# flo-audio/flo

Measured on AMD Instinct MI355X. Metric: Msamples/s encoded (44.1k stereo, q=high), higher is better.
Workload: dtype f32

## Files before the change

### flo_amd/csrc/batch.cpp

```cpp
#include <algorithm>
#include <chrono>
#include <cstdio>
#include <cstdlib>
#include <cstring>

#include "batch_internal.hpp"
#include "container_kernels.hpp"
#include "devpool.hpp"
#include "lossy_kernels.hpp"

static size_t lossy_max_frame_bytes(int ch) { return 12 + 50 * (size_t)ch + (size_t)ch * (4 + 2064); }

static LossyPlan lossy_plan(const flo_batch *b, int which, int force_path) {
    const char *tc = getenv("FLO_TAIL_CRC"), *clips = getenv("FLO_CHAIN2X_CLIPS");
    return plan_lossy({.which = which, .force_path = force_path, .ch = b->ch, .n_clips = b->n_clips, .total_frames = b->total_frames,
                       .exact = lossy_exact(b->exact != 0, b->ts->dev), .in_coeffs = b->d_in_coeffs != nullptr, .debug = b->d_dbg_coeffs || b->d_dbg_q || b->d_dbg_sfw,
                       .dirty = b->ts->dev.dirty, .tail_crc = !(tc && tc[0] == '0'), .chain2q_clips = clips ? atoi(clips) : 0});
}
static int alloc_frame_scratch(flo_batch *b, const LossyPlan &p) {
    flo_ctx *c = b->ctx;
    if (p.form != LossyForm::Frames || b->d_at || !b->total_frames) return FLO_OK;
    const size_t n = (size_t)b->total_frames * b->ch * 32 * sizeof(float);
    HIPCHK(c, pool_alloc(&b->d_at, n));
    HIPCHK(c, pool_alloc(&b->d_sprev, n));
// ... 312 lines not shown
    F.channels = b->ch;
    F.bit_depth = 16;
    F.level = 5;
    F.n_clips = (int)b->n_clips;
    F.crc_out = b->d_crc;
    F.part_reg = b->d_part;
    if (P.crc_ready) {
        F.crc_ready = b->d_crc_ready;
        F.epoch = b->epoch;
    }
    F.max_frames = max_frames;
    if ((rc = timed_launch(c, "finish_files", [&] { return launch_finish_files(F, fin, c->stream); })) != FLO_OK) return rc;
    if (P.crc_ready) {
        if (!b->pin_sizes) {
            std::string perr;
            if (!(b->pin_sizes = (uint64_t *)stager_pinned_get(c->stager, b->n_clips * 8, perr))) return fail(c, FLO_ERR_NOMEM, perr);
        }
        HIPCHK(c, hipMemcpyAsync(b->pin_sizes, b->d_clip_bytes, b->n_clips * 8, hipMemcpyDeviceToHost, c->stream));
        b->sizes_queued = true;
    }
    return FLO_OK;
}

extern "C" int flo_batch_encode(flo_batch *b, int which) {
    if (!b) return FLO_ERR_ARG;
    flo_ctx *c = b->ctx;
    if (which < 0 || which > 5) return fail(c, FLO_ERR_ARG, "unknown kernel form");
    HIPCHK(c, hipSetDevice(c->device));
    b->encoded = false;
    b->synced = false;
    if (b->mode == FLO_MODE_LOSSY) b->plan = lossy_plan(b, which, c->force_path);
    int erc = batch_encode_launch(b);
    b->encoded = erc == FLO_OK;
    b->encode_failed = erc != FLO_OK;
    return erc;
}

#ifdef FLO_STAMPS
static int stamps_report(flo_batch *b) {
    flo_ctx *c = b->ctx;
    if (!b->d_stamps || b->plan.form != LossyForm::Chain2q) return FLO_OK;
    std::vector<unsigned long long> st(b->n_clips * 2 * 16);
    HIPCHK(c, hipMemcpy(st.data(), b->d_stamps, st.size() * 8, hipMemcpyDeviceToHost));
    double t[14] = {0}, p[14] = {0};
    for (size_t k = 0; k < b->n_clips; k++)
        for (int i = 0; i < 14; i++) { t[i] += (double)st[(2 * k) * 16 + i]; p[i] += (double)st[(2 * k + 1) * 16 + i]; }
    static const char *tn[] = {"fold", "prefetch", "fft", "postrot", "bandstats", "mask", "quant", "wait-consumed", "handover"};
    static const char *pn[] = {"wait-ready", "read/quant", "pack0", "pack1", "flush", "wait-ts"};
    fprintf(stderr, "[stamps2x] ticks (10 ns) per stereo frame | T:");
    double tt = 0, pt = 0;
    for (int i = 0; i < 9; i++) { fprintf(stderr, " %s=%.1f", tn[i], t[i] / b->total_frames); tt += t[i]; }
    fprintf(stderr, " total=%.1f | P:", tt / b->total_frames);
    for (int i = 0; i < 6; i++) { fprintf(stderr, " %s=%.1f", pn[i], p[i] / b->total_frames); pt += p[i]; }
    fprintf(stderr, " total=%.1f item-form declined %.4f of channel-frames", pt / b->total_frames, p[6] / (2.0 * b->total_frames));
    fprintf(stderr, " | T waits>1000: %.2f%% of frames, %.0f cyc/frame avg; >5000: %.2f%%, %.0f | P busy>12000: %.2f%%, %.0f; >20000: %.2f%%, %.0f\n",
            100 * t[10] / b->total_frames, t[9] / b->total_frames, 100 * t[12] / b->total_frames, t[11] / b->total_frames,
            100 * p[10] / b->total_frames, p[9] / b->total_frames, 100 * p[12] / b->total_frames, p[11] / b->total_frames);
    std::vector<double> pb(b->n_clips), tb(b->n_clips);
    for (size_t k = 0; k < b->n_clips; k++) {
        const double fr = (double)b->hops[k] > 0 ? (double)b->hops[k] : 1.0;
        double tq = 0, pq = 0;
        for (int i = 0; i < 9; i++) if (i != 7) tq += (double)st[(2 * k) * 16 + i];
        for (int i = 1; i < 5; i++) pq += (double)st[(2 * k + 1) * 16 + i];
        tb[k] = tq / fr; pb[k] = pq / fr;
    }
    if (const char *dump = getenv("FLO_STAMPS_DUMP")) {
        if (FILE *fh = fopen(dump, "wb")) {
            fwrite(st.data(), 8, st.size(), fh);
            fclose(fh);
        }
    }
    std::vector<double> ps = pb, ts = tb;
    std::sort(ps.begin(), ps.end()); std::sort(ts.begin(), ts.end());
    fprintf(stderr, "[stamps2x] per-clip busy ticks per frame, deciles | P:");
    for (int d = 0; d <= 10; d++) fprintf(stderr, " %.0f", ps[std::min(b->n_clips - 1, (size_t)(d * (b->n_clips - 1) / 10))]);
    fprintf(stderr, " | T:");
    for (int d = 0; d <= 10; d++) fprintf(stderr, " %.0f", ts[std::min(b->n_clips - 1, (size_t)(d * (b->n_clips - 1) / 10))]);
    size_t pbound = 0;
    for (size_t k = 0; k < b->n_clips; k++) pbound += pb[k] > tb[k];
    fprintf(stderr, " | clips whose packer is busier than their transform: %.1f%%\n", 100.0 * pbound / b->n_clips);
    return FLO_OK;
}
#else
static int stamps_report(flo_batch *) { return FLO_OK; }
#endif

static int batch_sync_impl(flo_batch *b, hipEvent_t done) {
    flo_ctx *c = b->ctx;
    HIPCHK(c, hipSetDevice(c->device));
    if (done) HIPCHK(c, hipEventSynchronize(done));
    else HIPCHK(c, hipStreamSynchronize(c->stream));
    if (!b->encoded && b->encode_failed) return fail(c, FLO_ERR_STATE, "the last flo_batch_encode on this batch failed");
    if (b->encoded && !b->synced) {
        if (b->mode == FLO_MODE_LOSSY) {
            b->h_clip_bytes.assign(b->n_clips, 0);
            b->h_frame_size.clear();
            if (b->sizes_queued) {
                memcpy(b->h_clip_bytes.data(), b->pin_sizes, b->n_clips * 8);
            } else if (b->n_clips && b->total_frames) {
                if (done && c->down_stream) {
                    HIPCHK(c, hipMemcpyAsync(b->h_clip_bytes.data(), b->d_clip_bytes, b->n_clips * 8, hipMemcpyDeviceToHost, c->down_stream));
                    HIPCHK(c, hipStreamSynchronize(c->down_stream));
                } else {
                    HIPCHK(c, hipMemcpy(b->h_clip_bytes.data(), b->d_clip_bytes, b->n_clips * 8, hipMemcpyDeviceToHost));
                }
            }
            for (size_t i = 0; i < b->n_clips; i++)
// ... 365 lines not shown
```

### flo_amd/csrc/lossy_device.hpp

```cpp
#pragma once
#include <hip/hip_runtime.h>
#include <stdint.h>

#include "pack_rows.h"

namespace flo {


struct LossyDevTables {
    const float4 *pack;
    const float4 *pack_g;
    const float4 *pack_ext;
    const float *ath_db;
    const uint8_t *band;
    const float *band_count;
    const float *s10d;
    const uint32_t *lane_bnd;
    const uint32_t *lane_slot0;
    const uint32_t *band_slot0;
    int max_band_slots;
    uint32_t dirty;
    float smr_thr;
    int q_transparent;
};
// ... 1060 lines not shown
                                           const QuantRows &R, uint32_t (&xs)[2][8]) {
    typedef float v4f __attribute__((ext_vector_type(4)));
    typedef __attribute__((address_space(3))) v4f lds_f4;
    const uint32_t ts0 = (uint32_t)__builtin_amdgcn_readfirstlane((int)(uint32_t)(uintptr_t)ts);
    const uint32_t sgn_mask = 0x7FFFFFFFu;
    uint32_t phalf = 0x3EFFFFFFu;
    asm volatile("" : "+v"(phalf));
#pragma unroll
    for (int g = 0; g < 4; g++) {
        const float4 al4 = T.pack[(kRowAth + g) * 64 + lane];
        const float4 bo4 = R.bo4[g];
        const float al[4] = {al4.x, al4.y, al4.z, al4.w};
        const uint32_t bo[4] = {__float_as_uint(bo4.x), __float_as_uint(bo4.y), __float_as_uint(bo4.z), __float_as_uint(bo4.w)};
        v4f tb[4];
#pragma unroll
        for (int k = 0; k < 4; k++) tb[k] = *reinterpret_cast<const lds_f4 *>((uintptr_t)(ts0 + 2u * bo[k]));
        int v[2][4];
        float t[2][4];
#pragma unroll
        for (int k = 0; k < 4; k++) {
            const v2f x = c[4 * g + k];
            const v2f xsc = x * (v2f){tb[k].z, tb[k].w};
            uint32_t h0, h1;
            asm("v_bfi_b32 %0, %1, %2, %3" : "=v"(h0) : "s"(sgn_mask), "v"(phalf), "v"(x.x));
            asm("v_bfi_b32 %0, %1, %2, %3" : "=v"(h1) : "s"(sgn_mask), "v"(phalf), "v"(x.y));
            const v2f rs = xsc + (v2f){__uint_as_float(h0), __uint_as_float(h1)};
            v[0][k] = cvt_rz(rs.x);
            v[1][k] = cvt_rz(rs.y);
            t[0][k] = max_raw(tb[k].x, al[k]);
            t[1][k] = max_raw(tb[k].y, al[k]);
        }
#pragma unroll
        for (int ch = 0; ch < 2; ch++)
#pragma unroll
            for (int k2 = 0; k2 < 2; k2++) {
                const float xe = ch ? c[4 * g + 2 * k2].y : c[4 * g + 2 * k2].x;
                const float xo = ch ? c[4 * g + 2 * k2 + 1].y : c[4 * g + 2 * k2 + 1].x;
                uint32_t r;
                asm("v_cmp_gt_f32_e64 vcc, |%1|, %2\n\t"
                    "v_cndmask_b32_e32 %0, 0, %3, vcc\n\t"
                    "v_cmp_gt_f32_e64 vcc, |%4|, %5\n\t"
                    "v_cndmask_b32_sdwa %0, 0, %6, vcc dst_sel:WORD_1 dst_unused:UNUSED_PRESERVE src0_sel:DWORD src1_sel:DWORD"
                    : "=&v"(r)
                    : "v"(xe), "v"(t[ch][2 * k2]), "v"(v[ch][2 * k2]), "v"(xo), "v"(t[ch][2 * k2 + 1]), "v"(v[ch][2 * k2 + 1])
                    : "vcc");
                xs[ch][2 * g + k2] = r;
            }
    }
}

typedef float v4f __attribute__((ext_vector_type(4)));
template <int TSOFF>
__device__ __forceinline__ void quantise_nat(const v4f (&cf)[8], const uint32_t (&ts_a)[16], const float (&athn)[16],
                                             const uint32_t alive, const uint32_t (&blk)[8], uint32_t (&xd)[2][8]) {
    typedef __attribute__((address_space(3))) v4f lds_f4;
    const uint32_t sgn_mask = 0x7FFFFFFFu;
    uint32_t phalf = 0x3EFFFFFFu;
    asm volatile("" : "+v"(phalf));
    auto block = [&](const int k, const v4f t0, const v4f t1, uint32_t &out0, uint32_t &out1) __attribute__((always_inline)) {
        const v2f x0 = {cf[k].x, cf[k].y}, x1 = {cf[k].z, cf[k].w};
        const v2f s0 = x0 * (v2f){t0.z, t0.w}, s1 = x1 * (v2f){t1.z, t1.w};
        uint32_t h00, h01, h10, h11;
        asm("v_bfi_b32 %0, %1, %2, %3" : "=v"(h00) : "s"(sgn_mask), "v"(phalf), "v"(x0.x));
        asm("v_bfi_b32 %0, %1, %2, %3" : "=v"(h01) : "s"(sgn_mask), "v"(phalf), "v"(x0.y));
        asm("v_bfi_b32 %0, %1, %2, %3" : "=v"(h10) : "s"(sgn_mask), "v"(phalf), "v"(x1.x));
        asm("v_bfi_b32 %0, %1, %2, %3" : "=v"(h11) : "s"(sgn_mask), "v"(phalf), "v"(x1.y));
        const v2f r0 = s0 + (v2f){__uint_as_float(h00), __uint_as_float(h01)};
        const v2f r1 = s1 + (v2f){__uint_as_float(h10), __uint_as_float(h11)};
        const int v0[2] = {cvt_rz(r0.x), cvt_rz(r0.y)}, v1[2] = {cvt_rz(r1.x), cvt_rz(r1.y)};
        const float a0 = athn[2 * k], a1 = athn[2 * k + 1];
        const float th0[2] = {max_raw(t0.x, a0), max_raw(t0.y, a0)}, th1[2] = {max_raw(t1.x, a1), max_raw(t1.y, a1)};
        uint32_t r[2];
#pragma unroll
        for (int ch = 0; ch < 2; ch++) {
            const float xe = ch ? x0.y : x0.x, xo = ch ? x1.y : x1.x;
            asm("v_cmp_gt_f32_e64 vcc, |%1|, %2\n\t"
                "v_cndmask_b32_e32 %0, 0, %3, vcc\n\t"
                "v_cmp_gt_f32_e64 vcc, |%4|, %5\n\t"
                "v_cndmask_b32_sdwa %0, 0, %6, vcc dst_sel:WORD_1 dst_unused:UNUSED_PRESERVE src0_sel:DWORD src1_sel:DWORD"
                : "=&v"(r[ch])
                : "v"(xe), "v"(th0[ch]), "v"(v0[ch]), "v"(xo), "v"(th1[ch]), "v"(v1[ch])
                : "vcc");
        }
        out0 = r[0];
        out1 = r[1];
    };
#pragma unroll
    for (int g = 0; g < 4; g++) {
        uint32_t o00 = 0u, o01 = 0u, o10 = 0u, o11 = 0u;
        if (alive & (blk[2 * g] | blk[2 * g + 1])) {
            v4f tb[4];
#pragma unroll
            for (int j = 0; j < 4; j++) tb[j] = *reinterpret_cast<const lds_f4 *>((uintptr_t)(ts_a[4 * g + j] + (uint32_t)TSOFF));
            if (alive & blk[2 * g]) block(2 * g, tb[0], tb[1], o00, o01);
            if (alive & blk[2 * g + 1]) block(2 * g + 1, tb[2], tb[3], o10, o11);
        }
        xd[0][2 * g] = o00, xd[1][2 * g] = o01;
        xd[0][2 * g + 1] = o10, xd[1][2 * g + 1] = o11;
    }
}

__device__ __forceinline__ uint32_t nonzero_mask16(const int (&q)[16]) {
    uint32_t m = 0;
#pragma unroll
    for (int e = 0; e < 16; e++) m |= (q[e] != 0 ? 1u : 0u) << e;
    return m;
}
__device__ __forceinline__ uint32_t nonzero_mask16_packed(const uint32_t (&x)[8], const uint32_t (&hi)[8]) {
    uint32_t m = 0;
#pragma unroll
    for (int k = 0; k < 8; k++) {
        m |= ((x[k] & 0xFFFFu) != 0u ? 1u : 0u) << (2 * k);
        m |= (hi[k] != 0u ? 1u : 0u) << (2 * k + 1);
    }
    return m;
}
__device__ __forceinline__ uint32_t wave_incl_sum(uint32_t x) {
    int v = (int)x;
    v += dpp_i<0x111>(0, v);
    v += dpp_i<0x112>(0, v);
    v += dpp_i<0x114>(0, v);
    v += dpp_i<0x118>(0, v);
    v += dpp_i<0x142, 0xA>(0, v);
    v += dpp_i<0x143, 0xC>(0, v);
    return (uint32_t)v;
}

struct SparsePlan {
    uint32_t M;
    int nn;
    int nz_end;
    uint32_t cross_cnt;
    uint32_t off0;
    uint32_t total;
};

__device__ __forceinline__ void sparse_plan_m(const int lane, const uint32_t m, SparsePlan &P) {
    const uint32_t prev_m = (uint32_t)dpp_i<0x138>(0, (int)m);
    const uint32_t prev_nz = (prev_m >> 15) & 1u;
    uint32_t zs = ~m & ((m << 1) | prev_nz) & 0xFFFFu;
    if (lane == 0 && !(m & 1u)) zs |= 1u;
    const int base = 16 * lane;
    const uint32_t inv = ~m & 0xFFFFu;
    const int first_nz = m ? base + __builtin_ctz(m) : 1024;
    const int first_z = inv ? base + __builtin_ctz(inv) : 1024;
    const int last_z = inv ? base + 31 - __builtin_clz(inv) : -1;
    const unsigned long long has_nz = __ballot(m != 0u), has_z = __ballot(inv != 0u);
    const unsigned long long nz_above = (has_nz >> 1) >> lane, z_above = (has_z >> 1) >> lane;
// ... 86 lines not shown
    while (any) {
        any = 0;
#pragma unroll
        for (int c = 0; c < CH; c++) {
            const bool active = CH == 1 || hm[c] != 0u;
            const int s = __builtin_ctz(hm[c] | 0x10000u);
            hm[c] &= hm[c] - 1;
            any |= hm[c];
            const uint32_t below = (1u << s) - 1u;
            const uint32_t off = P[c].off0 + 2u * (uint32_t)__builtin_popcount(P[c].M & (below | (below << 16)));
            const uint32_t above = m[c] >> s;
            const bool leaves = above == 0u;
            const int zin = (int)__builtin_ctz(above | 0x10000u);
            const uint32_t zc = leaves ? (uint32_t)(nn_rel[c] - s) : (uint32_t)zin;
            const int e = s + zin;
            const int run = __builtin_ctz(~(m[c] >> (e & 15)));
            const int len = (e + run >= 16) ? nzend_rel[c] - e : run;
            uint32_t cnt = (uint32_t)(len < 255 ? len : 255);
            cnt = leaves ? P[c].cross_cnt : cnt;
            const bool wide = zc >= 128u;
            const uint32_t o = active ? off : trash_off[c];
            dst[c][o] = (uint8_t)(wide ? ((zc & 0x7Fu) | 0x80u) : zc);
            dst[c][o + 1] = (uint8_t)(wide ? (zc >> 7) : cnt);
            dst[c][(wide && active) ? off + 2 : trash_off[c]] = (uint8_t)cnt;
        }
    }
#pragma unroll
    for (int i = 0; i < 16; i++) {
#pragma unroll
        for (int c = 0; c < CH; c++) {
            const uint32_t K = ((1u << i) - 1u) | (((2u << i) - 1u) << 16);
            const uint32_t off = P[c].off0 + 2u * (uint32_t)__builtin_popcount(P[c].M & K);
            const uint32_t o = ((m[c] >> i) & 1u) ? off : trash_off[c];
            const uint32_t v = (uint32_t)q[c][i];
            dst[c][o] = (uint8_t)v;
            dst[c][o + 1] = (uint8_t)(v >> 8);
        }
    }
}

constexpr int kRunTabEntries = 128;
constexpr uint32_t kSparseFallback = 0xFFFFFFFFu;

__device__ __forceinline__ void lds_st8_at(uint32_t a, uint32_t v, const int off) {
    if (off == 0) asm volatile("ds_write_b8 %0, %1" ::"v"(a), "v"(v) : "memory");
    else if (off == 1) asm volatile("ds_write_b8 %0, %1 offset:1" ::"v"(a), "v"(v) : "memory");
    else if (off == 2) asm volatile("ds_write_b8 %0, %1 offset:2" ::"v"(a), "v"(v) : "memory");
    else asm volatile("ds_write_b8 %0, %1 offset:3" ::"v"(a), "v"(v) : "memory");
}
__device__ __forceinline__ uint32_t mbcnt64(unsigned long long m) {
    return __builtin_amdgcn_mbcnt_hi((uint32_t)(m >> 32), __builtin_amdgcn_mbcnt_lo((uint32_t)m, 0u));
}

__device__ __forceinline__ uint32_t sparse_block_pack(const int lane, const uint32_t (&xd)[8], const uint32_t blob, const uint32_t tab) {
    uint32_t nM = 0, nS = 0, W = 0, cz = 0;
    unsigned long long carry = 0;
    const uint32_t tmax = tab + 4u * (uint32_t)(kRunTabEntries - 1);
    const uint32_t pos_l = (uint32_t)(2 * lane);
#pragma unroll
    for (int k = 0; k < 8; k++) {
        unsigned long long E;
        asm("v_cmp_ne_u16_e64 %0, 0, %1" : "=s"(E) : "v"(xd[k]));
        const unsigned long long O = __ballot(xd[k] > 0xFFFFu);
        const unsigned long long any = E | O;
        if (any == 0ull) {
            cz += 128u;
            carry = 0;
            continue;
        }
        {
            uint32_t t, nf;
            asm("s_ff1_i32_b64 %0, %2\n\ts_bitcmp1_b64 %3, %0\n\ts_cselect_b32 %1, 0, 1" : "=&s"(t), "=s"(nf) : "s"(any), "s"(E) : "scc");
            W += cz + 2u * t + nf >= 128u ? 1u : 0u;
        }
        const unsigned long long S_lo = E & ~((O << 1) | carry), S_hi = O & ~E, S = S_lo | S_hi;
        carry = O >> 63;
        {
            uint32_t fl, nb;
            asm("s_flbit_i32_b64 %0, %2\n\ts_sub_u32 %1, 63, %0\n\ts_bitcmp1_b64 %3, %1\n\ts_cselect_b32 %1, 0, 1"
                : "=&s"(fl), "=&s"(nb) : "s"(any), "s"(O) : "scc");
            cz = 2u * fl + nb;
        }
        const uint32_t nzb = __builtin_amdgcn_mbcnt_hi((uint32_t)(O >> 32), __builtin_amdgcn_mbcnt_lo((uint32_t)O, mbcnt64(E)));
        const uint32_t stb = mbcnt64(S);
        uint32_t slo, shi;
        asm("v_cndmask_b32_e64 %0, 0, 1, %1" : "=v"(slo) : "s"(S_lo));
        asm("v_cndmask_b32_e64 %0, 0, 1, %1" : "=v"(shi) : "s"(S_hi));
        const uint32_t a = ((nzb + stb + slo) << 1) + (blob + W + 2u * (nM + nS));
        uint32_t ta = (stb << 2) + (tab + 4u * (nS + 1u));
        ta = ta < tmax ? ta : tmax;
        const uint32_t ent = (nzb << 16) + ((nM << 16) + (uint32_t)(128 * k)) + (pos_l + shi);
        {
            const uint32_t x8 = xd[k] >> 8;
            unsigned long long sv;
            asm volatile("s_mov_b64 %0, exec\n\t"
                         "s_mov_b64 exec, %1\n\tds_write_b8 %4, %5\n\tds_write_b8 %4, %6 offset:1\n\t"
                         "s_mov_b64 exec, %2\n\tds_write_b8_d16_hi %4, %5 offset:2\n\tds_write_b8_d16_hi %4, %6 offset:3\n\t"
                         "s_mov_b64 exec, %3\n\tds_write_b32 %7, %8\n\t"
                         "s_mov_b64 exec, %0"
                         : "=&s"(sv)
                         : "s"(E), "s"(O), "s"(S), "v"(a), "v"(xd[k]), "v"(x8), "v"(ta), "v"(ent));
        }
        nM += (uint32_t)__builtin_popcountll(E) + (uint32_t)__builtin_popcountll(O);
        nS += (uint32_t)__builtin_popcountll(S);
    }
    const uint32_t N = nM, R = nS;
    if (N == 0u) {
        if (lane == 0) {
            lds_st8_at(blob, 0x80u, 0);
            lds_st8_at(blob, 0x08u, 1);
            lds_st8_at(blob, 0u, 2);
        }
        return 3u;
// ... 4 lines not shown
        asm volatile("ds_write_b32 %0, %1" ::"v"(tab + 4u * (R + 1u)), "v"(N << 16) : "memory");
    }
    uint32_t wdone = 0;
    bool too_long = false;
    for (uint32_t j0 = 0; j0 < R; j0 += 64u) {
        const uint32_t j = j0 + (uint32_t)lane;
        const bool act = j < R;
        const uint32_t ja = tab + 4u * (act ? j : 0u);
        uint32_t e0, e1, e2;
        asm volatile("ds_read_b32 %0, %3\n\tds_read_b32 %1, %3 offset:4\n\tds_read_b32 %2, %3 offset:8\n\ts_waitcnt lgkmcnt(0)"
                     : "=&v"(e0), "=&v"(e1), "=&v"(e2)
                     : "v"(ja)
                     : "memory");
        const uint32_t p0 = e0 & 0xFFFFu, r0 = e0 >> 16, p1 = e1 & 0xFFFFu, r1 = e1 >> 16, r2 = e2 >> 16;
        const uint32_t cnt = r2 - r1;
        const uint32_t zrun = p1 - (p0 + (r1 - r0));
        const bool wide = act && zrun >= 128u;
        const unsigned long long wb = __ballot(wide);
        too_long |= __ballot(act && cnt > 255u) != 0ull;
        uint32_t wex = wdone;
        if (wb != 0ull) {
            wex += mbcnt64(wb);
            wdone += (uint32_t)__builtin_popcountll(wb);
        }
        const uint32_t ha = ((r1 + j) << 1) + (blob + wex);
        if (act) {
            lds_st8_at(ha, wide ? ((zrun & 0x7Fu) | 0x80u) : zrun, 0);
            lds_st8_at(ha, wide ? (zrun >> 7) : cnt, 1);
            if (wide) lds_st8_at(ha, cnt, 2);
        }
    }
    if (too_long) return kSparseFallback;
    uint32_t tot = 2u * (N + R) + W;
    if (cz != 0u) {
        const uint32_t ta = blob + tot;
        if (lane == 0) {
            if (cz >= 128u) {
                lds_st8_at(ta, (cz & 0x7Fu) | 0x80u, 0);
                lds_st8_at(ta, cz >> 7, 1);
                lds_st8_at(ta, 0u, 2);
            } else {
                lds_st8_at(ta, cz, 0);
                lds_st8_at(ta, 0u, 1);
            }
        }
        tot += cz >= 128u ? 3u : 2u;
    }
    return tot;
}

constexpr int kItemCap = 128;
constexpr int kItemTbl = 136;
constexpr int kPackTabDwords = 272;
__device__ __forceinline__ uint32_t sparse_item_pack(const int lane, const uint32_t (&xd)[8], const uint32_t blob, const uint32_t tabp) {
    typedef __attribute__((address_space(3))) uint32_t lds_u32;
    const uint32_t list1 = tabp + 4u;
    const uint32_t pk0 = (uint32_t)(2 * lane + 1) << 16;
    if (lane == 0) asm volatile("ds_write_b32 %0, %1" ::"v"(tabp), "v"(0u) : "memory");
    uint32_t nM = 0;
#pragma unroll
    for (int k = 0; k < 8; k++) {
        unsigned long long E;
        asm("v_cmp_ne_u16_e64 %0, 0, %1" : "=s"(E) : "v"(xd[k]));
        const unsigned long long O = __ballot(xd[k] > 0xFFFFu);
        if ((E | O) == 0ull) continue;
        uint32_t re = __builtin_amdgcn_mbcnt_hi((uint32_t)(O >> 32), __builtin_amdgcn_mbcnt_lo((uint32_t)O,
                      __builtin_amdgcn_mbcnt_hi((uint32_t)(E >> 32), __builtin_amdgcn_mbcnt_lo((uint32_t)E, nM))));
        re = re < (uint32_t)kItemCap ? re : (uint32_t)kItemCap;
        const uint32_t a_e = (re << 2) + list1;
        uint32_t e4;
        asm("v_cndmask_b32_e64 %0, 0, 4, %1" : "=v"(e4) : "s"(E));
        const uint32_t a_o = a_e + e4;
        const uint32_t pk_e = pk0 + ((uint32_t)k << 23);
        uint32_t it_e;
        asm("v_bfi_b32 %0, %1, %2, %3" : "=v"(it_e) : "s"(0xFFFFu), "v"(xd[k]), "v"(pk_e));
        const uint32_t it_o = __builtin_amdgcn_perm(pk_e + 0x10000u, xd[k], 0x07060302u);
        unsigned long long sv;
        asm volatile("s_mov_b64 %0, exec\n\t"
                     "s_mov_b64 exec, %1\n\tds_write_b32 %3, %4\n\t"
                     "s_mov_b64 exec, %2\n\tds_write_b32 %5, %6\n\t"
                     "s_mov_b64 exec, %0"
                     : "=&s"(sv)
                     : "s"(E), "s"(O), "v"(a_e), "v"(it_e), "v"(a_o), "v"(it_o)
                     : "memory");
        nM += (uint32_t)__builtin_popcountll(E) + (uint32_t)__builtin_popcountll(O);
    }
    const uint32_t N = nM;
    if (N > (uint32_t)kItemCap) return kSparseFallback;
    wave_sync();
    const uint32_t vaddr = tabp + 4u * (uint32_t)lane;
    const uint32_t tblp = tabp + 4u * (uint32_t)kItemTbl;
    const uint32_t lane2 = 2u * (uint32_t)lane;
    const uint32_t b3 = blob - 3u;
    const bool two = N > 64u;
    const uint32_t prevA = *reinterpret_cast<const lds_u32 *>((uintptr_t)vaddr), itA = *reinterpret_cast<const lds_u32 *>((uintptr_t)(vaddr + 4u));
    uint32_t diffA;
    asm("v_sub_u32_sdwa %0, %1, %2 dst_sel:DWORD dst_unused:UNUSED_PAD src0_sel:WORD_1 src1_sel:WORD_1" : "=v"(diffA) : "v"(itA), "v"(prevA));
    const unsigned long long maskA = N >= 64u ? ~0ull : ((1ull << N) - 1ull);
    const unsigned long long SmA = (__ballot(diffA != 1u) | 1ull) & maskA;
    const unsigned long long WmA = __ballot(diffA >= 129u) & SmA;
    uint32_t ownA, ownWA;
    asm("v_cndmask_b32_e64 %0, 0, 1, %1" : "=v"(ownA) : "s"(SmA));
    asm("v_cndmask_b32_e64 %0, 0, 1, %1" : "=v"(ownWA) : "s"(WmA));
    const uint32_t rA = __builtin_amdgcn_mbcnt_hi((uint32_t)(SmA >> 32), __builtin_amdgcn_mbcnt_lo((uint32_t)SmA, ownA));
    const uint32_t wA = __builtin_amdgcn_mbcnt_hi((uint32_t)(WmA >> 32), __builtin_amdgcn_mbcnt_lo((uint32_t)WmA, ownWA));
    const uint32_t baseA = ((rA << 1) + wA) + (lane2 + b3);
    const uint32_t RA = (uint32_t)__builtin_popcountll(SmA), WA = (uint32_t)__builtin_popcountll(WmA);
    {
        unsigned long long sv;
        asm volatile("s_mov_b64 %0, exec\n\ts_mov_b64 exec, %1\n\tds_write_b32 %2, %3\n\ts_mov_b64 exec, %0"
                     : "=&s"(sv) : "s"(SmA), "v"((rA << 2) + tblp), "v"((uint32_t)lane) : "memory");
    }
    uint32_t itB = 0, diffB = 1, rB = 0, baseB = 0, RB = 0, WB = 0;
    unsigned long long maskB = 0, SmB = 0, WmB = 0;
// ... 83 lines not shown
```

### flo_amd/csrc/lossy_kernels.hip

```cpp
#include <assert.h>
#include <stdlib.h>

#include <mutex>
#include <set>
#include <type_traits>
#include <utility>

#include "chain2q_roles.hpp"
#include "crc_device.hpp"
#include "lossy_device.hpp"
#include "lossy_kernels.hpp"
#include "../../include/flo_synth.h"

#ifndef FLO_SKIP
#define FLO_SKIP 0
#endif
#define FLO_KEEP(x) asm volatile("" ::"v"(x))
#ifdef FLO_STAMPS
#define STAMP(i)                                                                                  \
    do {                                                                                          \
        __builtin_amdgcn_sched_barrier(0);                                                        \
        unsigned long long t_;                                                                    \
        asm volatile("s_memtime %0\n\ts_waitcnt lgkmcnt(0)" : "=s"(t_)::"memory");              \
        __builtin_amdgcn_sched_barrier(0);                                                        \
// ... 384 lines not shown
        }
        const unsigned tag = (unsigned)__builtin_amdgcn_readfirstlane((int)(unsigned)(e >> 32));
        clip = (unsigned)__builtin_amdgcn_readfirstlane((int)(unsigned)e);
        if (tag != A.epoch || clip >= (unsigned)A.n_clips) return;
        __builtin_amdgcn_fence(__ATOMIC_ACQUIRE, "agent");
        asm volatile("s_waitcnt vmcnt(0)" ::: "memory");
        total = __hip_atomic_load(A.clip_bytes + clip, __ATOMIC_RELAXED, __HIP_MEMORY_SCOPE_AGENT);
    }
}

constexpr int kPackerPrio = 1;
constexpr unsigned kPackerTurns = 1;
template <bool COEFFS, uint32_t DIRTY, bool DBG>
__global__ __launch_bounds__(FLO_C2X_THREADS) void lossy_chain2q_kernel(LossyArgs A, int clips_per_wg, const StatMasks *__restrict__ masks) {
    extern __shared__ __attribute__((aligned(16))) uint8_t lds_raw[];
    const int tid = (int)threadIdx.x;
    const int lane = tid & 63;
    {
        float4 *dstp = reinterpret_cast<float4 *>(lds_raw);
        for (int i = tid; i < kPackRowsHotT * 64; i += (int)blockDim.x) dstp[i] = A.T.pack[i];
        for (int i = tid; i < clips_per_wg; i += (int)blockDim.x) {
            Clip2qLds &c0 = *reinterpret_cast<Clip2qLds *>(lds_raw + kPackBytesHotT + (size_t)i * sizeof(Clip2qLds));
            c0.coef_ready = 0;
            c0.ts_ready = 0;
            c0.consumed = 0;
            c0.clip_seq = 0;
        }
        if (A.clear_next && blockIdx.x == 0 && tid == 0)
            A.clear_next[0] = A.clear_next[1] = A.clear_next[2] = 0;
    }
    __syncthreads();
    const int wv = __builtin_amdgcn_readfirstlane(tid >> 6);
    const Chain2qRole role = chain2q_role(clips_per_wg, wv);
    const int cl = role.slot;
    Clip2qLds &cs = *reinterpret_cast<Clip2qLds *>(lds_raw + kPackBytesHotT + (size_t)cl * sizeof(Clip2qLds));
    uint32_t fbase = 0, seq = 0;
    if (role.packer) {
        __builtin_amdgcn_s_setprio(kPackerPrio);
        const uint32_t pturn = A.chain2q_pturns && chain2q_peers_on_simd(clips_per_wg, wv) > 1 ? 1u + (uint32_t)(chain2q_rank_on_simd(clips_per_wg, wv) & 1) : 0u;
        typedef __attribute__((address_space(3))) v4f lds_v4f;
        float athn[16];
        uint32_t ts_a[16];
        {
            const uint32_t ts0 = (uint32_t)(uintptr_t)cs.ts[0];
#pragma unroll
            for (int q = 0; q < 4; q++) {
                const float4 a4 = A.T.pack[(kRowAthN + q) * 64 + lane];
                const float4 b4 = A.T.pack[(kRowBoN + q) * 64 + lane];
                athn[4 * q + 0] = a4.x, athn[4 * q + 1] = a4.y, athn[4 * q + 2] = a4.z, athn[4 * q + 3] = a4.w;
                ts_a[4 * q + 0] = ts0 + __float_as_uint(b4.x), ts_a[4 * q + 1] = ts0 + __float_as_uint(b4.y);
                ts_a[4 * q + 2] = ts0 + __float_as_uint(b4.z), ts_a[4 * q + 3] = ts0 + __float_as_uint(b4.w);
            }
        }
        const uint32_t *const blk_g = reinterpret_cast<const uint32_t *>(A.T.pack + kRowBlk * 64);
        const uint32_t cf_a = (uint32_t)(uintptr_t)cs.u.coef2 + 16u * (uint32_t)lane + 16u * ((uint32_t)lane >> 3);
        uint8_t *const stage = cs.stage;
        const uint32_t tab_a = (uint32_t)(uintptr_t)cs.packtab;
        v4f cf[8];
        bool have = false;
        unsigned done_clip = ~0u;
        unsigned long long done_bytes = 0;
        for (;;) {
            unsigned got = 0;
            if (lane == 0) got = atomicAdd(A.next_clip, 1u);
            const unsigned clip = (unsigned)__builtin_amdgcn_readfirstlane((int)got);
            if (lane == 0) cs.clip_cur = clip;
            set_counter(&cs.clip_seq, ++seq);
            if (A.crc_ready) {
                if (clip >= (unsigned)A.n_clips) {
                    tail_crc(A, reinterpret_cast<uint32_t *>(&cs.u), lane, done_clip, done_bytes);
                    return;
                }
                if (done_clip != ~0u) tail_publish(A, done_clip, lane);
            }
            if (clip >= (unsigned)A.n_clips) return;
            const unsigned hops = A.clip_hops[clip];
            const unsigned long long frame0 = A.clip_frame0[clip];
            uint8_t *gout = A.out + A.out_off[clip];
            unsigned long long written = 0;
            uint32_t pend = 0, tailb = 0;
            STAMPS_BEGIN();
            for (unsigned h = 0; h < hops; h++) {
                const int ln = lane_id_opaque();
                const uint32_t g = fbase + h;
                if (pturn) {
                    if ((h + pturn) & 1u) __builtin_amdgcn_s_setprio(kPackerPrio);
                    else __builtin_amdgcn_s_setprio(kPackerPrio + 1);
                }
                auto take_next = [&]() __attribute__((always_inline)) {
                    if (!have && (uint32_t)__builtin_amdgcn_readfirstlane((int)peek_counter(&cs.coef_ready)) >= g + 2) {
#pragma unroll
                        for (int k = 0; k < 8; k++) cf[k] = *reinterpret_cast<const lds_v4f *>((uintptr_t)(cf_a + 1152u * (uint32_t)k));
                        set_counter(&cs.consumed, g + 2);
                        have = true;
                    }
                };
                uint32_t blk[8];
                {
                    const uint32_t *bp = blk_g;
                    asm volatile("" : "+s"(bp));
#pragma unroll
                    for (int q = 0; q < 8; q++) blk[q] = bp[q];
                }
                if (!have) {
                    wait_counter(&cs.coef_ready, g + 1);
#pragma unroll
                    for (int k = 0; k < 8; k++) cf[k] = *reinterpret_cast<const lds_v4f *>((uintptr_t)(cf_a + 1152u * (uint32_t)k));
                    set_counter(&cs.consumed, g + 1);
                }
                STAMP(0);
#ifdef FLO_STAMPS
                const unsigned long long st_frame0 = st_last;
#endif
                wait_counter(&cs.ts_ready, g + 1);
                STAMP(5);
                const uint32_t par = g & 1u;
                const uint32_t sfw_both = cs.sfwh[par][ln >> 5][ln & 31];
                const uint32_t alive = (uint32_t)__builtin_amdgcn_readfirstlane((int)(cs.alive[par][0] | cs.alive[par][1]));
                uint32_t xd[2][8];
#if (FLO_SKIP & 64) == 0
                if (par) quantise_nat<512>(cf, ts_a, athn, alive, blk, xd);
                else quantise_nat<0>(cf, ts_a, athn, alive, blk, xd);
#else
#pragma unroll
                for (int q = 0; q < 8; q++) { xd[0][q] = __float_as_uint(cf[q].x) & alive & 0x00010001u; xd[1][q] = __float_as_uint(cf[q].y) & blk[q] & 0x00010001u; }
#endif
                have = false;
                take_next();
                STAMP(1);
                if (DBG && A.dbg_q) {
#pragma unroll
                    for (int ch = 0; ch < 2; ch++) {
                        uint32_t *dq = reinterpret_cast<uint32_t *>(A.dbg_q + ((frame0 + h) * 2 + ch) * 1024);
#pragma unroll
                        for (int k = 0; k < 8; k++) dq[64 * k + ln] = xd[ch][k];
                    }
                }
                if (ln < (int)pend) stage[ln] = (uint8_t)tailb;
                uint8_t *f = stage + pend;
                const uint32_t f_a = (uint32_t)(uintptr_t)f;
                if ((ln & 31) < 25) {
                    uint8_t *p = f + 12 + 50 * (ln >> 5) + 2 * (ln & 31);
                    lds_st8<0>(p, sfw_both);
                    lds_st8<1>(p, sfw_both >> 8);
                }
                uint32_t tot[2];
                uint32_t pos = 112;
#pragma unroll
                for (int ch = 0; ch < 2; ch++) {
#if (FLO_SKIP & 32) == 0
                    uint32_t t = sparse_item_pack(ln, xd[ch], f_a + pos + 4u, tab_a);
#ifdef FLO_STAMPS
                    if (t == kSparseFallback) st_sum[6] += 1;
#endif
                    if (t == kSparseFallback) t = sparse_block_pack(ln, xd[ch], f_a + pos + 4u, tab_a);
#else
                    uint32_t t = 3u + ((xd[ch][0] | xd[ch][3]) & 1u);
                    FLO_KEEP(xd[ch][1]); FLO_KEEP(xd[ch][2]); FLO_KEEP(xd[ch][4]); FLO_KEEP(xd[ch][5]); FLO_KEEP(xd[ch][6]); FLO_KEEP(xd[ch][7]);
#endif
                    if (t == kSparseFallback) {
                        uint32_t *scr = reinterpret_cast<uint32_t *>(stage + 2560);
#pragma unroll
                        for (int k = 0; k < 8; k++) scr[64 * k + ln] = xd[ch][k];
                        wave_sync();
                        const uint4 x0 = reinterpret_cast<const uint4 *>(scr)[2 * ln], x1 = reinterpret_cast<const uint4 *>(scr)[2 * ln + 1];
                        wave_sync();
                        const uint32_t xs[8] = {x0.x, x0.y, x0.z, x0.w, x1.x, x1.y, x1.z, x1.w};
                        int q[1][16];
                        uint32_t hi[8];
#pragma unroll
                        for (int k = 0; k < 8; k++) {
                            hi[k] = xs[k] >> 16;
                            q[0][2 * k] = (int)xs[k];
                            q[0][2 * k + 1] = (int)hi[k];
                        }
                        SparsePlan P[1];
                        sparse_plan_m(ln, nonzero_mask16_packed(xs, hi), P[0]);
                        uint8_t *const dsts[1] = {f + pos + 4};
                        const uint32_t trash[1] = {(uint32_t)((stage + kFrameCap + 64 + 2 * ln) - dsts[0])};
                        sparse_emit_n<1>(ln, q, P, dsts, trash);
                        t = P[0].total;
                    }
                    tot[ch] = t;
                    pos += 4u + t;
                    if (ch == 0) take_next();
                    STAMP(2 + ch);
                }
                const uint32_t flen = pos, blob_len = flen - 10;
                {
                    const uint32_t i = (uint32_t)ln;
                    const uint32_t w0 = 0x000400FDu, w1 = blob_len << 16, w2 = (blob_len >> 16) | 0x02000000u;
                    uint32_t wv4 = i < 4u ? w0 : (i < 8u ? w1 : w2);
                    wv4 = i < 12u ? wv4 : (i < 16u ? tot[0] : tot[1]);
                    const uint32_t off = i < 12u ? i : (i < 16u ? 112u - 12u + i : 116u - 16u + tot[0] + i);
                    const uint32_t bv = wv4 >> (8u * (i & 3u));
                    if (i < 20u) lds_st8<0>(f + off, bv);
                    if (ln == 0) A.frame_size[frame0 + h] = flen;
                }
                wave_sync();
                take_next();
                const uint32_t haveb = pend + flen;
                const uint32_t n16 = haveb >> 4;
                const uint4 *src = reinterpret_cast<const uint4 *>(stage);
                uint4 *dst = reinterpret_cast<uint4 *>(gout + written);
                for (uint32_t i = ln; i < n16; i += 64) dst[i] = src[i];
                pend = haveb & 15u;
                tailb = (ln < (int)pend) ? stage[(n16 << 4) + ln] : 0u;
                written += (unsigned long long)n16 << 4;
                wave_sync();
                STAMP(4);
#ifdef FLO_STAMPS
                {
                    const unsigned long long busy = st_last - st_frame0;
                    if (busy > 12000) { st_sum[9] += busy; st_sum[10] += 1; }
                    if (busy > 20000) { st_sum[11] += busy; st_sum[12] += 1; }
                }
#endif
            }
            if (lane < (int)pend) gout[written + lane] = (uint8_t)tailb;
            if (lane == 0) A.clip_bytes[clip] = written + pend;
            done_clip = clip;
            done_bytes = written + pend;
            STAMPS_RECORD(1);
            fbase += hops;
        }
    }

    LossyDevTables T = A.T;
    T.pack = reinterpret_cast<const float4 *>(lds_raw);
    uint32_t so_pre[12], slot_first;
    band_stats_2_prepare(lane, cs.slot, A.T.pack, so_pre, slot_first);
    unsigned long long close[16];
    band_stats_2_masks<DIRTY>(masks, close);
    v4f tw[4];
    if (!COEFFS) {
#pragma unroll
        for (int k = 0; k < 4; k++) tw[k] = pack_row_v(&T.pack[(kRowTw + k) * 64 + lane]);
    }
    for (;;) {
        wait_counter(&cs.clip_seq, ++seq);
        const unsigned clip = (unsigned)__builtin_amdgcn_readfirstlane((int)cs.clip_cur);
        if (clip >= (unsigned)A.n_clips) return;
        const unsigned hops = A.clip_hops[clip];
        const unsigned long long frame0 = A.clip_frame0[clip];
        const float *pcm = A.pcm + A.clip_off[clip];

        float prev = 0.f;
        v2f ne[8], no[8], acar[8];
        if (!COEFFS) {
            fold_carry_init_2(lane_id_opaque(), acar, T);
            load_half_fast_2(lane_id_opaque(), pcm, 0, ne, no);
        }
        STAMPS_BEGIN();
        v2f zr[8], zi[8];
        if (!COEFFS) fold_carry_2(lane_id_opaque(), ne, no, acar, tw, zr, zi, T);
        float pend_e = 0.f, pend_m = 0.f;
        auto mask_publish = [&](const int ln, const uint32_t gp, const unsigned hp, const float energy1, const float bmax1,
                                const float rcount, const float4 sd0, const float4 sd1) __attribute__((always_inline)) {
            const int bnd = ln & 31, up = ln >> 5;
#if (FLO_SKIP & 16) == 0
            const float bm = bmax1;
            const float sfv1 = bm > 1e-10f ? __fdiv_rn(30000.0f, bm) : 1.0f;
            const uint32_t sfw1 = sf_word(sfv1);
            const float a = spread_threshold_2r(ln, energy1, rcount, sd0, sd1, T);
            const float sl = max_raw(a, prev * 0.7f);
            prev = sl;
            const float tl1 = masking_amplitude(sl, T.smr_thr);
#else
            const float bm = bmax1, tl1 = energy1 * 1e-3f + rcount + sd0.x + sd1.y, sfv1 = bm * 100.f + 1.f;
            const uint32_t sfw1 = __float_as_uint(tl1) >> 16;
#endif
            const unsigned long long al = __ballot(bnd < 25 && bm > tl1);
            if (bnd < 25) {
                typedef __attribute__((address_space(3))) float lds_f32;
                const uint32_t ts_s = (uint32_t)__builtin_amdgcn_readfirstlane((int)(uint32_t)(uintptr_t)cs.ts[gp & 1u]);
                lds_f32 *tp = reinterpret_cast<lds_f32 *>((uintptr_t)(ts_s + 16u * (uint32_t)bnd + 4u * (uint32_t)up));
                tp[0] = tl1;
                tp[2] = sfv1;
                cs.sfwh[gp & 1u][up][bnd] = (uint16_t)sfw1;
            }
            if (ln == 0) {
                cs.alive[gp & 1u][0] = (uint32_t)al;
                cs.alive[gp & 1u][1] = (uint32_t)(al >> 32);
            }
            if (DBG && A.dbg_sfw && bnd < 25) A.dbg_sfw[((frame0 + hp) * 2 + up) * 25 + bnd] = (unsigned short)sfw1;
            set_counter(&cs.ts_ready, gp + 1);
        };
        auto frame_body = [&](const unsigned h) __attribute__((always_inline)) {
            const int ln = lane_id_opaque();
            const uint32_t g = fbase + h;
            FLO_MARK("frame_begin");
            const uint32_t consumed_early = peek_counter(&cs.consumed);
            const float4 sd0 = T.pack[kRowS10 * 64], sd1 = T.pack[kRowS10 * 64 + 1];
            const float rcount = reinterpret_cast<const float *>(T.pack + kRowS10 * 64)[64 + ln];
            v2f c[16];
            if (COEFFS) {
#pragma unroll
                for (int q = 0; q < 4; q++) {
                    const float4 v0 = reinterpret_cast<const float4 *>(A.in_coeffs + ((frame0 + h) * 2 + 0) * 1024 + 16 * ln)[q];
                    const float4 v1 = reinterpret_cast<const float4 *>(A.in_coeffs + ((frame0 + h) * 2 + 1) * 1024 + 16 * ln)[q];
                    c[4 * q] = (v2f){v0.x, v1.x}; c[4 * q + 1] = (v2f){v0.y, v1.y};
                    c[4 * q + 2] = (v2f){v0.z, v1.z}; c[4 * q + 3] = (v2f){v0.w, v1.w};
                }
                if ((uint32_t)__builtin_amdgcn_readfirstlane((int)consumed_early) < g) wait_counter(&cs.consumed, g);
                float4 *p = reinterpret_cast<float4 *>(&cs.u.coef2[18 * ln]);
#pragma unroll
                for (int q = 0; q < 8; q++) p[q] = make_float4(c[2 * q].x, c[2 * q].y, c[2 * q + 1].x, c[2 * q + 1].y);
                wave_sync();
            } else {
                load_half_fast_2(ln, pcm, (long long)(h + 1) * 1024, ne, no);
                FLO_MARK("prefetch_done");
                STAMP(1);
                if ((uint32_t)__builtin_amdgcn_readfirstlane((int)consumed_early) < g) wait_counter(&cs.consumed, g);
                STAMP(7);
#if (FLO_SKIP & 8) == 0
                fft512_2(ln, zr, zi, cs.u.xch4, T, [&]() __attribute__((always_inline)) {
                    if (h > 0) mask_publish(ln, g - 1u, h - 1u, pend_e, pend_m, rcount, sd0, sd1);
                });
#else
                if (h > 0) mask_publish(ln, g - 1u, h - 1u, pend_e, pend_m, rcount, sd0, sd1);
#endif
                FLO_MARK("fft_done");
                STAMP(2);
#if (FLO_SKIP & 4) == 0
                post_rotate_transpose_2_tw(ln, zr, zi, cs.u.coef2, c, tw);
// ... 1025 lines not shown
```

### flo_amd/csrc/pack_rows.h

```cpp
#pragma once

namespace flo {
constexpr int kRowWin = 0;
constexpr int kRowTw = 8;
constexpr int kRowF1 = 12;
constexpr int kRowF2 = 16;
constexpr int kRowLane = 20;
constexpr int kRowKeep = 21;
constexpr int kRowDst = 25;
constexpr int kRowLst = 29;
constexpr int kRowS10 = 32;
constexpr int kPackRowsHotT = 33;
constexpr int kRowAth = 33;
constexpr int kRowBo = 37;
constexpr int kPackRowsHot = 41;
constexpr int kRowLstCold = 41;
constexpr int kRowAthN = 44;
constexpr int kRowBoN = 48;
constexpr int kRowBlk = 52;
constexpr int kPackRows = 53;

struct StatMasks {
    unsigned long long close[16];
    unsigned long long gather[3];
};
}
```

### flo_amd/csrc/tables.cpp

```cpp
#include "tables.hpp"

#include "pack_rows.h"

#include <cmath>
#include <cstring>

namespace flo {

static const int kSlotCapHost = 96;

static const float kPi = 3.14159265358979323846f;

static const float kBarkEdges[26] = {0.0f,    100.0f,  200.0f,  300.0f,  400.0f,  510.0f,   630.0f,
                                     770.0f,  920.0f,  1080.0f, 1270.0f, 1480.0f, 1720.0f,  2000.0f,
                                     2320.0f, 2700.0f, 3150.0f, 3700.0f, 4400.0f, 5300.0f,  6400.0f,
                                     7700.0f, 9500.0f, 12000.0f, 15500.0f, 20500.0f};

float ref_ath(float freq) {
    if (!(freq >= 20.0f && freq <= 20000.0f)) return 96.0f;
    float f_khz = freq / 1000.0f;
    float term1 = 3.64f * powf(f_khz, -0.8f);
    float d = f_khz - 3.3f;
    float term2 = 6.5f * expf(-0.6f * (d * d));
    float f2 = f_khz * f_khz;
// ... 140 lines not shown
    }
    t.band_slot0[kNumBands] = (uint32_t)s;
    t.max_band_slots = 0;
    for (int b = 0; b < kNumBands; b++) {
        int n = (int)(t.band_slot0[b + 1] - t.band_slot0[b]);
        if (n > t.max_band_slots) t.max_band_slots = n;
    }
    auto PU = [&](int row, int lane, int i, uint32_t v) { memcpy(&t.pack[((size_t)row * 64 + lane) * 4 + i], &v, 4); };
    for (int lane = 0; lane < 64; lane++) {
        const int bl = lane & 31;
        const int b = bl < 25 ? bl : 24;
        const float cnt = t.band_count[b];
        const float rcount = cnt > 0.f ? 1.0f / cnt : 0.f;
        uint32_t rc;
        memcpy(&rc, &rcount, 4);
        const uint32_t bs0 = t.band_slot0[b] + (uint32_t)(lane >> 5);
        const uint32_t bs1 = bl < 25 ? t.band_slot0[b + 1] : 0u;
        {
            uint32_t slot = t.lane_slot0[lane];
            for (int e = 0; e < 16; e++) {
                const bool end = (t.lane_bnd[lane] >> e) & 1u;
                PU(kRowBo + e / 4, lane, e % 4, (uint32_t)t.band[16 * lane + e] * 8u);
                P(kRowKeep + e / 4, lane, e % 4) = end ? 0.0f : 1.0f;
                PU(kRowDst + e / 4, lane, e % 4, (end ? slot : (uint32_t)(kSlotCapHost + lane)) * 8u);
                if (end) slot++;
            }
        }
        for (int u = 0; u < 24; u++) {
            const uint32_t sidx = bs0 + 2u * (uint32_t)u;
            PU((u < 12 ? kRowLst : kRowLstCold - 3) + u / 4, lane, u % 4, (sidx < bs1 ? sidx : (uint32_t)(kSlotCapHost + 64)) * 8u);
        }
        for (int u = 24; u < 32; u++) {
            const uint32_t sidx = bs0 + 2u * (uint32_t)u;
            const uint32_t v = (sidx < bs1 ? sidx : (uint32_t)(kSlotCapHost + 64)) * 8u;
            memcpy(&t.pack_ext[((size_t)((u - 24) / 4) * 64 + lane) * 4 + u % 4], &v, 4);
        }
        for (int e = 0; e < 16; e++) PU(kRowBoN + e / 4, lane, e % 4, (uint32_t)t.band[128 * (e >> 1) + 2 * lane + (e & 1)] * 16u);
        PU(kRowLane, lane, 0, t.lane_bnd[lane]);
        PU(kRowLane, lane, 1, t.lane_slot0[lane]);
        PU(kRowLane, lane, 2, rc);
        PU(kRowS10, 16 + lane / 4, lane % 4, rc);
        PU(kRowLane, lane, 3, bs0 | (bs1 << 16));
    }
    t.masks = StatMasks{};
    for (int lane = 0; lane < 64; lane++) {
        for (int e = 0; e < 16; e++)
            if ((t.lane_bnd[lane] >> e) & 1u) t.masks.close[e] |= 1ull << lane;
        const int bl = lane & 31;
        const uint32_t bs0 = t.band_slot0[bl < 25 ? bl : 24] + (uint32_t)(lane >> 5), bs1 = bl < 25 ? t.band_slot0[bl + 1] : 0u;
        const uint32_t n = bs0 < bs1 ? (bs1 - bs0 + 1u) / 2u : 0u;
        for (int g = 0; g < 3; g++)
            if (n > 4u * (uint32_t)g) t.masks.gather[g] |= 1ull << lane;
    }
    uint32_t nonzero = 0;
    for (int e = 0; e < 16; e++) nonzero |= (t.masks.close[e] != 0) << e;
    t.masks_ok = nonzero == t.dirty && t.masks.close[15] == ~0ull && t.n_slots <= kSlotCapHost;
}

}
```

Before: 702,400.

## Skip quantise and pack for blocks with no bands above the ATH floor

Result: faster. 710,700 (median of 6 runs) (+1.2%).

```diff
diff --git a/flo_amd/csrc/batch.cpp b/flo_amd/csrc/batch.cpp
--- a/flo_amd/csrc/batch.cpp
+++ b/flo_amd/csrc/batch.cpp
@@ -388,7 +388,8 @@
     for (int i = 0; i < 9; i++) { fprintf(stderr, " %s=%.1f", tn[i], t[i] / b->total_frames); tt += t[i]; }
     fprintf(stderr, " total=%.1f | P:", tt / b->total_frames);
     for (int i = 0; i < 6; i++) { fprintf(stderr, " %s=%.1f", pn[i], p[i] / b->total_frames); pt += p[i]; }
-    fprintf(stderr, " total=%.1f item-form declined %.4f of channel-frames", pt / b->total_frames, p[6] / (2.0 * b->total_frames));
+    fprintf(stderr, " total=%.1f item-form declined %.4f of channel-frames, blocks quantised per frame %.3f", pt / b->total_frames,
+            p[6] / (2.0 * b->total_frames), p[7] / b->total_frames);
     fprintf(stderr, " | T waits>1000: %.2f%% of frames, %.0f cyc/frame avg; >5000: %.2f%%, %.0f | P busy>12000: %.2f%%, %.0f; >20000: %.2f%%, %.0f\n",
             100 * t[10] / b->total_frames, t[9] / b->total_frames, 100 * t[12] / b->total_frames, t[11] / b->total_frames,
             100 * p[10] / b->total_frames, p[9] / b->total_frames, 100 * p[12] / b->total_frames, p[11] / b->total_frames);
diff --git a/flo_amd/csrc/lossy_device.hpp b/flo_amd/csrc/lossy_device.hpp
--- a/flo_amd/csrc/lossy_device.hpp
+++ b/flo_amd/csrc/lossy_device.hpp
@@ -1136,7 +1136,7 @@
 typedef float v4f __attribute__((ext_vector_type(4)));
 template <int TSOFF>
 __device__ __forceinline__ void quantise_nat(const v4f (&cf)[8], const uint32_t (&ts_a)[16], const float (&athn)[16],
-                                             const uint32_t alive, const uint32_t (&blk)[8], uint32_t (&xd)[2][8]) {
+                                             const uint32_t visit, uint32_t (&xd)[2][8]) {
     typedef __attribute__((address_space(3))) v4f lds_f4;
     const uint32_t sgn_mask = 0x7FFFFFFFu;
     uint32_t phalf = 0x3EFFFFFFu;
@@ -1169,15 +1169,24 @@
         out0 = r[0];
         out1 = r[1];
     };
+    uint32_t va = visit, vb = visit;
+    asm volatile("" : "+s"(va));
+    asm volatile("" : "+s"(vb));
 #pragma unroll
     for (int g = 0; g < 4; g++) {
         uint32_t o00 = 0u, o01 = 0u, o10 = 0u, o11 = 0u;
-        if (alive & (blk[2 * g] | blk[2 * g + 1])) {
+        if ((va >> (2 * g)) & 3u) {
             v4f tb[4];
-#pragma unroll
-            for (int j = 0; j < 4; j++) tb[j] = *reinterpret_cast<const lds_f4 *>((uintptr_t)(ts_a[4 * g + j] + (uint32_t)TSOFF));
-            if (alive & blk[2 * g]) block(2 * g, tb[0], tb[1], o00, o01);
-            if (alive & blk[2 * g + 1]) block(2 * g + 1, tb[2], tb[3], o10, o11);
+            if ((va >> (2 * g)) & 1u) {
+                tb[0] = *reinterpret_cast<const lds_f4 *>((uintptr_t)(ts_a[4 * g + 0] + (uint32_t)TSOFF));
+                tb[1] = *reinterpret_cast<const lds_f4 *>((uintptr_t)(ts_a[4 * g + 1] + (uint32_t)TSOFF));
+            }
+            if ((va >> (2 * g + 1)) & 1u) {
+                tb[2] = *reinterpret_cast<const lds_f4 *>((uintptr_t)(ts_a[4 * g + 2] + (uint32_t)TSOFF));
+                tb[3] = *reinterpret_cast<const lds_f4 *>((uintptr_t)(ts_a[4 * g + 3] + (uint32_t)TSOFF));
+            }
+            if ((vb >> (2 * g)) & 1u) block(2 * g, tb[0], tb[1], o00, o01);
+            if ((vb >> (2 * g + 1)) & 1u) block(2 * g + 1, tb[2], tb[3], o10, o11);
         }
         xd[0][2 * g] = o00, xd[1][2 * g] = o01;
         xd[0][2 * g + 1] = o10, xd[1][2 * g + 1] = o11;
@@ -1370,13 +1379,19 @@
     return __builtin_amdgcn_mbcnt_hi((uint32_t)(m >> 32), __builtin_amdgcn_mbcnt_lo((uint32_t)m, 0u));
 }
 
-__device__ __forceinline__ uint32_t sparse_block_pack(const int lane, const uint32_t (&xd)[8], const uint32_t blob, const uint32_t tab) {
+__device__ __forceinline__ uint32_t sparse_block_pack(const int lane, const uint32_t (&xd)[8], const uint32_t blob, const uint32_t tab,
+                                                      const uint32_t visited = 0xFFu) {
     uint32_t nM = 0, nS = 0, W = 0, cz = 0;
     unsigned long long carry = 0;
     const uint32_t tmax = tab + 4u * (uint32_t)(kRunTabEntries - 1);
     const uint32_t pos_l = (uint32_t)(2 * lane);
 #pragma unroll
     for (int k = 0; k < 8; k++) {
+        if (!((visited >> k) & 1u)) {
+            cz += 128u;
+            carry = 0;
+            continue;
+        }
         unsigned long long E;
         asm("v_cmp_ne_u16_e64 %0, 0, %1" : "=s"(E) : "v"(xd[k]));
         const unsigned long long O = __ballot(xd[k] > 0xFFFFu);
@@ -1487,7 +1502,8 @@
 constexpr int kItemCap = 128;
 constexpr int kItemTbl = 136;
 constexpr int kPackTabDwords = 272;
-__device__ __forceinline__ uint32_t sparse_item_pack(const int lane, const uint32_t (&xd)[8], const uint32_t blob, const uint32_t tabp) {
+__device__ __forceinline__ uint32_t sparse_item_pack(const int lane, const uint32_t (&xd)[8], const uint32_t blob, const uint32_t tabp,
+                                                     const uint32_t visited = 0xFFu) {
     typedef __attribute__((address_space(3))) uint32_t lds_u32;
     const uint32_t list1 = tabp + 4u;
     const uint32_t pk0 = (uint32_t)(2 * lane + 1) << 16;
@@ -1495,6 +1511,7 @@
     uint32_t nM = 0;
 #pragma unroll
     for (int k = 0; k < 8; k++) {
+        if (!((visited >> k) & 1u)) continue;
         unsigned long long E;
         asm("v_cmp_ne_u16_e64 %0, 0, %1" : "=s"(E) : "v"(xd[k]));
         const unsigned long long O = __ballot(xd[k] > 0xFFFFu);
diff --git a/flo_amd/csrc/lossy_kernels.hip b/flo_amd/csrc/lossy_kernels.hip
--- a/flo_amd/csrc/lossy_kernels.hip
+++ b/flo_amd/csrc/lossy_kernels.hip
@@ -460,7 +460,8 @@
                 ts_a[4 * q + 2] = ts0 + __float_as_uint(b4.z), ts_a[4 * q + 3] = ts0 + __float_as_uint(b4.w);
             }
         }
-        const uint32_t *const blk_g = reinterpret_cast<const uint32_t *>(A.T.pack + kRowBlk * 64);
+        uint32_t blk_l = reinterpret_cast<const uint32_t *>(A.T.pack + kRowBlk * 64)[lane & 7];
+        asm volatile("" : "+v"(blk_l));
         const uint32_t cf_a = (uint32_t)(uintptr_t)cs.u.coef2 + 16u * (uint32_t)lane + 16u * ((uint32_t)lane >> 3);
         uint8_t *const stage = cs.stage;
         const uint32_t tab_a = (uint32_t)(uintptr_t)cs.packtab;
@@ -503,13 +504,6 @@
                         have = true;
                     }
                 };
-                uint32_t blk[8];
-                {
-                    const uint32_t *bp = blk_g;
-                    asm volatile("" : "+s"(bp));
-#pragma unroll
-                    for (int q = 0; q < 8; q++) blk[q] = bp[q];
-                }
                 if (!have) {
                     wait_counter(&cs.coef_ready, g + 1);
 #pragma unroll
@@ -527,11 +521,16 @@
                 const uint32_t alive = (uint32_t)__builtin_amdgcn_readfirstlane((int)(cs.alive[par][0] | cs.alive[par][1]));
                 uint32_t xd[2][8];
 #if (FLO_SKIP & 64) == 0
-                if (par) quantise_nat<512>(cf, ts_a, athn, alive, blk, xd);
-                else quantise_nat<0>(cf, ts_a, athn, alive, blk, xd);
+                const uint32_t visited = (uint32_t)__ballot((alive & blk_l) != 0u) & 0xFFu;
+                if (par) quantise_nat<512>(cf, ts_a, athn, visited, xd);
+                else quantise_nat<0>(cf, ts_a, athn, visited, xd);
 #else
-#pragma unroll
-                for (int q = 0; q < 8; q++) { xd[0][q] = __float_as_uint(cf[q].x) & alive & 0x00010001u; xd[1][q] = __float_as_uint(cf[q].y) & blk[q] & 0x00010001u; }
+                const uint32_t visited = 0xFFu;
+#pragma unroll
+                for (int q = 0; q < 8; q++) { xd[0][q] = __float_as_uint(cf[q].x) & alive & 0x00010001u; xd[1][q] = __float_as_uint(cf[q].y) & blk_l & 0x00010001u; }
+#endif
+#ifdef FLO_STAMPS
+                st_sum[7] += (unsigned long long)__builtin_popcount(visited);
 #endif
                 have = false;
                 take_next();
@@ -557,11 +556,11 @@
 #pragma unroll
                 for (int ch = 0; ch < 2; ch++) {
 #if (FLO_SKIP & 32) == 0
-                    uint32_t t = sparse_item_pack(ln, xd[ch], f_a + pos + 4u, tab_a);
+                    uint32_t t = sparse_item_pack(ln, xd[ch], f_a + pos + 4u, tab_a, visited);
 #ifdef FLO_STAMPS
                     if (t == kSparseFallback) st_sum[6] += 1;
 #endif
-                    if (t == kSparseFallback) t = sparse_block_pack(ln, xd[ch], f_a + pos + 4u, tab_a);
+                    if (t == kSparseFallback) t = sparse_block_pack(ln, xd[ch], f_a + pos + 4u, tab_a, visited);
 #else
                     uint32_t t = 3u + ((xd[ch][0] | xd[ch][3]) & 1u);
                     FLO_KEEP(xd[ch][1]); FLO_KEEP(xd[ch][2]); FLO_KEEP(xd[ch][4]); FLO_KEEP(xd[ch][5]); FLO_KEEP(xd[ch][6]); FLO_KEEP(xd[ch][7]);
@@ -640,6 +639,8 @@
     band_stats_2_prepare(lane, cs.slot, A.T.pack, so_pre, slot_first);
     unsigned long long close[16];
     band_stats_2_masks<DIRTY>(masks, close);
+    float ath_floor = masks->band_ath_floor[lane & 31];
+    asm volatile("" : "+v"(ath_floor));
     v4f tw[4];
     if (!COEFFS) {
 #pragma unroll
@@ -678,7 +679,7 @@
             const float bm = bmax1, tl1 = energy1 * 1e-3f + rcount + sd0.x + sd1.y, sfv1 = bm * 100.f + 1.f;
             const uint32_t sfw1 = __float_as_uint(tl1) >> 16;
 #endif
-            const unsigned long long al = __ballot(bnd < 25 && bm > tl1);
+            const unsigned long long al = __ballot(bnd < 25 && bm > tl1 && bm > ath_floor);
             if (bnd < 25) {
                 typedef __attribute__((address_space(3))) float lds_f32;
                 const uint32_t ts_s = (uint32_t)__builtin_amdgcn_readfirstlane((int)(uint32_t)(uintptr_t)cs.ts[gp & 1u]);
diff --git a/flo_amd/csrc/pack_rows.h b/flo_amd/csrc/pack_rows.h
--- a/flo_amd/csrc/pack_rows.h
+++ b/flo_amd/csrc/pack_rows.h
@@ -23,5 +23,6 @@
 struct StatMasks {
     unsigned long long close[16];
     unsigned long long gather[3];
+    float band_ath_floor[32];
 };
 }
diff --git a/flo_amd/csrc/tables.cpp b/flo_amd/csrc/tables.cpp
--- a/flo_amd/csrc/tables.cpp
+++ b/flo_amd/csrc/tables.cpp
@@ -216,6 +216,11 @@
         for (int g = 0; g < 3; g++)
             if (n > 4u * (uint32_t)g) t.masks.gather[g] |= 1ull << lane;
     }
+    for (int b = 0; b < 32; b++) t.masks.band_ath_floor[b] = INFINITY;
+    for (int k = 0; k < kHop; k++) {
+        float &f = t.masks.band_ath_floor[t.band[k]];
+        if (t.ath_lin[k] < f) f = t.ath_lin[k];
+    }
     uint32_t nonzero = 0;
     for (int e = 0; e < 16; e++) nonzero |= (t.masks.close[e] != 0) << e;
     t.masks_ok = nonzero == t.dirty && t.masks.close[15] == ~0ull && t.n_slots <= kSlotCapHost;
```
